# MiNeves00/SR-GAN-FD

Hardware: AMD Instinct MI355X
Metric: SR training images/sec (128->512 x4, f16) (higher is better)
Workload: dtype f16; 1 GPU; BSRGAN RRDBNet x4 generator-only (L1), 23 RRDB, batch 32/GPU, 128->512; global_batch=32, num_rrdb=23, parallelism=dp1

## Files before the change

sr_gan_fd_amd/csrc/pack.hip:

```cpp
#include "common.hpp"

namespace srganfd {

__global__ __launch_bounds__(256) void pack_kernel(const srganfd_pack_job* __restrict__ jobs, const float* __restrict__ params,
                                                   const float* __restrict__ scalars, char* __restrict__ packed) {
  const srganfd_pack_job& J = jobs[blockIdx.y];
  const int KT = J.ksize * J.ksize;
  const long long total = (long long)KT * J.k * J.n;
  const int nChunks = J.k >> 5;
  for (long long e = (long long)blockIdx.x * 256 + threadIdx.x; e < total; e += (long long)gridDim.x * 256) {
    int lane, s, k_in, within = (int)(e & 1023);
    long long blk = e >> 10;
    const int tap = (int)(blk % KT); blk /= KT;
    const int chunk = (int)(blk % nChunks);
    const int ntile = (int)(blk / nChunks);
    int n_in = -1;
    if (J.dtype != SRGANFD_F32 && J.layout == 1) {
      const int j = within & 7; lane = (within >> 3) & 63; s = within >> 9;
      k_in = 8 * (lane >> 4) + j;
      n_in = 16 * s + (lane & 15);
    } else if (J.dtype != SRGANFD_F32) {
      const int j = within & 7; lane = (within >> 3) & 63; s = within >> 9;
      k_in = 16 * s + 8 * (lane >> 5) + j;
    } else {
      lane = within & 63; s = within >> 6;
      k_in = 2 * s + (lane >> 5);
    }
    const int k = chunk * 32 + k_in, n = ntile * 32 + (n_in >= 0 ? n_in : (lane & 31));
    float v = 0.f;
    for (int g = 0; g < J.nseg; ++g) {
      const srganfd_pack_seg& S = J.seg[g];
      if (k >= S.k_lo && k < S.k_lo + S.k_len) {
        const int kk = k - S.k_lo;
        int co, ci, t = 0;
        int KTs = KT;
        int ym = 0, xm = 0;
        if (!S.transposed) { co = n + S.co_off; ci = kk + S.ci_off; t = tap; }
        else if (S.transposed == 1) { co = kk + S.co_off; ci = n + S.ci_off; t = KT - 1 - tap; }
        else if (S.transposed < 6) {
          const int py = (S.transposed - 2) >> 1, px = (S.transposed - 2) & 1, ta = tap >> 1, tb = tap & 1;
          const int ty = py ? 2 - 2 * ta : 3 - 2 * ta, tx = px ? 2 - 2 * tb : 3 - 2 * tb;
          co = kk + S.co_off; ci = n + S.ci_off; t = ty * 4 + tx; KTs = 16;
        } else if (S.transposed < 10) {
          const int py = (S.transposed - 6) >> 1, px = (S.transposed - 6) & 1, ta = tap >> 1, tb = tap & 1;
          const int ty = py ? (ta ? 0 : 2) : (ta ? -1 : 1), tx = px ? (tb ? 0 : 2) : (tb ? -1 : 1);
          co = kk + S.co_off; ci = n + S.ci_off; KTs = 9;
          t = ty * 3 + tx;
          if (ty < 0 || tx < 0) co = S.co_src;
        } else if (S.transposed < 14) {
          const int ab = S.transposed - 10;
          co = kk + S.co_off; ci = n + S.ci_off; t = ab; KTs = 4;
        } else if (S.transposed < 18) {
          const int py = (S.transposed - 14) >> 1, px = (S.transposed - 14) & 1, ta = tap >> 1, tb = tap & 1;
          co = n + S.co_off; ci = kk + S.ci_off; KTs = 9;
          ym = py ? (ta ? 4 : 3) : (ta ? 6 : 1);
          xm = px ? (tb ? 4 : 3) : (tb ? 6 : 1);
        } else {
          const int u = tap >> 2, w = tap & 3;
          co = kk + S.co_off; ci = n + S.ci_off; KTs = 9;
          ym = (0x1364 >> (4 * u)) & 7;
          xm = (0x1364 >> (4 * w)) & 7;
        }
        if (co < S.co_src && ci < S.ci_src) {
          const float* src = params + S.src_off + ((long long)co * S.ci_src + ci) * KTs;
          if (ym) {
            float sum = 0.f;
            for (int ty = 0; ty < 3; ++ty)
              for (int tx = 0; tx < 3; ++tx)
                if ((ym >> ty) & (xm >> tx) & 1) sum += src[ty * 3 + tx];
            v = sum * S.scale;
          } else {
            v = src[t] * S.scale;
          }
          if (S.scale_off >= 0) v *= scalars[S.scale_off];
        }
        break;
      }
    }
    if (J.dtype == SRGANFD_BF16) ((bf16_t*)(packed + J.dst_off))[e] = f2bf(v);
    else if (J.dtype == SRGANFD_F16) ((f16_t*)(packed + J.dst_off))[e] = (f16_t)v;
    else ((float*)(packed + J.dst_off))[e] = v;
  }
}

extern "C" size_t srganfd_packed_bytes(int32_t dtype, int32_t ksize, int32_t k, int32_t n) {
  if (k <= 0 || n <= 0 || k % 32 || n % 32) return 0;
  return (size_t)ksize * ksize * k * n * (dtype == SRGANFD_F32 ? 4 : 2);
}
extern "C" int srganfd_pack_weights(const srganfd_pack_job* jobs_dev, int32_t njobs, int64_t max_elems, const float* params,
                                    const float* scalars, void* packed, void* stream) {
  if (!jobs_dev || njobs <= 0 || max_elems <= 0 || !params || !packed) return set_err(SRGANFD_EINVAL, "pack_weights: bad args");
  long long gx = (max_elems + 255) / 256;
  if (gx > 4096) gx = 4096;
  SRGANFD_LAUNCH(pack_kernel, dim3((unsigned)gx, (unsigned)njobs), dim3(256), 0, (hipStream_t)stream, jobs_dev, params, scalars, (char*)packed);
  SRGANFD_HIP_CHECK(hipGetLastError());
  return SRGANFD_OK;
}

}
```

Before: 551.4 img/s.

## Tile weight packing through shared memory with coalesced source loads and vector stores

The weight pack kernel now processes one 32x32 (k,n) block per workgroup. It stages the source weight rows for that block into LDS with coalesced reads, then emits 16-byte vectorized stores per thread. The goal is to replace the scattered per-element global gathers of the fp32 master weights during each step's repack. It adds LDS use and two barriers per block, and changes the grid sizing. An environment variable can turn the tiling off.

```diff
diff --git a/sr_gan_fd_amd/csrc/pack.hip b/sr_gan_fd_amd/csrc/pack.hip
--- a/sr_gan_fd_amd/csrc/pack.hip
+++ b/sr_gan_fd_amd/csrc/pack.hip
@@ -1,87 +1,168 @@
 #include "common.hpp"
+#include <cstdlib>
 
 namespace srganfd {
 
-__global__ __launch_bounds__(256) void pack_kernel(const srganfd_pack_job* __restrict__ jobs, const float* __restrict__ params,
-                                                   const float* __restrict__ scalars, char* __restrict__ packed) {
-  const srganfd_pack_job& J = jobs[blockIdx.y];
-  const int KT = J.ksize * J.ksize;
-  const long long total = (long long)KT * J.k * J.n;
-  const int nChunks = J.k >> 5;
-  for (long long e = (long long)blockIdx.x * 256 + threadIdx.x; e < total; e += (long long)gridDim.x * 256) {
-    int lane, s, k_in, within = (int)(e & 1023);
-    long long blk = e >> 10;
-    const int tap = (int)(blk % KT); blk /= KT;
-    const int chunk = (int)(blk % nChunks);
-    const int ntile = (int)(blk / nChunks);
-    int n_in = -1;
-    if (J.dtype != SRGANFD_F32 && J.layout == 1) {
-      const int j = within & 7; lane = (within >> 3) & 63; s = within >> 9;
-      k_in = 8 * (lane >> 4) + j;
-      n_in = 16 * s + (lane & 15);
-    } else if (J.dtype != SRGANFD_F32) {
-      const int j = within & 7; lane = (within >> 3) & 63; s = within >> 9;
-      k_in = 16 * s + 8 * (lane >> 5) + j;
-    } else {
-      lane = within & 63; s = within >> 6;
-      k_in = 2 * s + (lane >> 5);
-    }
-    const int k = chunk * 32 + k_in, n = ntile * 32 + (n_in >= 0 ? n_in : (lane & 31));
-    float v = 0.f;
-    for (int g = 0; g < J.nseg; ++g) {
-      const srganfd_pack_seg& S = J.seg[g];
-      if (k >= S.k_lo && k < S.k_lo + S.k_len) {
-        const int kk = k - S.k_lo;
-        int co, ci, t = 0;
-        int KTs = KT;
-        int ym = 0, xm = 0;
-        if (!S.transposed) { co = n + S.co_off; ci = kk + S.ci_off; t = tap; }
-        else if (S.transposed == 1) { co = kk + S.co_off; ci = n + S.ci_off; t = KT - 1 - tap; }
-        else if (S.transposed < 6) {
-          const int py = (S.transposed - 2) >> 1, px = (S.transposed - 2) & 1, ta = tap >> 1, tb = tap & 1;
-          const int ty = py ? 2 - 2 * ta : 3 - 2 * ta, tx = px ? 2 - 2 * tb : 3 - 2 * tb;
-          co = kk + S.co_off; ci = n + S.ci_off; t = ty * 4 + tx; KTs = 16;
-        } else if (S.transposed < 10) {
-          const int py = (S.transposed - 6) >> 1, px = (S.transposed - 6) & 1, ta = tap >> 1, tb = tap & 1;
-          const int ty = py ? (ta ? 0 : 2) : (ta ? -1 : 1), tx = px ? (tb ? 0 : 2) : (tb ? -1 : 1);
-          co = kk + S.co_off; ci = n + S.ci_off; KTs = 9;
-          t = ty * 3 + tx;
-          if (ty < 0 || tx < 0) co = S.co_src;
-        } else if (S.transposed < 14) {
-          const int ab = S.transposed - 10;
-          co = kk + S.co_off; ci = n + S.ci_off; t = ab; KTs = 4;
-        } else if (S.transposed < 18) {
-          const int py = (S.transposed - 14) >> 1, px = (S.transposed - 14) & 1, ta = tap >> 1, tb = tap & 1;
-          co = n + S.co_off; ci = kk + S.ci_off; KTs = 9;
-          ym = py ? (ta ? 4 : 3) : (ta ? 6 : 1);
-          xm = px ? (tb ? 4 : 3) : (tb ? 6 : 1);
-        } else {
-          const int u = tap >> 2, w = tap & 3;
-          co = kk + S.co_off; ci = n + S.ci_off; KTs = 9;
-          ym = (0x1364 >> (4 * u)) & 7;
-          xm = (0x1364 >> (4 * w)) & 7;
-        }
-        if (co < S.co_src && ci < S.ci_src) {
-          const float* src = params + S.src_off + ((long long)co * S.ci_src + ci) * KTs;
-          if (ym) {
+static constexpr int kPackTileTaps = 9;
+static constexpr int kPackRow = 32 * kPackTileTaps + 1;
+
+__device__ __forceinline__ void pack_pos(int dtype, int layout, int within, int& k_in, int& n_in) {
+  if (dtype != SRGANFD_F32 && layout == 1) {
+    const int j = within & 7, lane = (within >> 3) & 63, s = within >> 9;
+    k_in = 8 * (lane >> 4) + j;
+    n_in = 16 * s + (lane & 15);
+  } else if (dtype != SRGANFD_F32) {
+    const int j = within & 7, lane = (within >> 3) & 63, s = within >> 9;
+    k_in = 16 * s + 8 * (lane >> 5) + j;
+    n_in = lane & 31;
+  } else {
+    const int lane = within & 63, s = within >> 6;
+    k_in = 2 * s + (lane >> 5);
+    n_in = lane & 31;
+  }
+}
+
+struct PackSrc { int co, ci, t, KTs, ym, xm; };
+__device__ __forceinline__ PackSrc pack_source(const srganfd_pack_seg& S, int KT, int tap, int kk, int n) {
+  PackSrc P;
+  P.t = 0; P.KTs = KT; P.ym = 0; P.xm = 0;
+  if (!S.transposed) { P.co = n + S.co_off; P.ci = kk + S.ci_off; P.t = tap; }
+  else if (S.transposed == 1) { P.co = kk + S.co_off; P.ci = n + S.ci_off; P.t = KT - 1 - tap; }
+  else if (S.transposed < 6) {
+    const int py = (S.transposed - 2) >> 1, px = (S.transposed - 2) & 1, ta = tap >> 1, tb = tap & 1;
+    const int ty = py ? 2 - 2 * ta : 3 - 2 * ta, tx = px ? 2 - 2 * tb : 3 - 2 * tb;
+    P.co = kk + S.co_off; P.ci = n + S.ci_off; P.t = ty * 4 + tx; P.KTs = 16;
+  } else if (S.transposed < 10) {
+    const int py = (S.transposed - 6) >> 1, px = (S.transposed - 6) & 1, ta = tap >> 1, tb = tap & 1;
+    const int ty = py ? (ta ? 0 : 2) : (ta ? -1 : 1), tx = px ? (tb ? 0 : 2) : (tb ? -1 : 1);
+    P.co = kk + S.co_off; P.ci = n + S.ci_off; P.KTs = 9;
+    P.t = ty * 3 + tx;
+    if (ty < 0 || tx < 0) P.co = S.co_src;
+  } else if (S.transposed < 14) {
+    const int ab = S.transposed - 10;
+    P.co = kk + S.co_off; P.ci = n + S.ci_off; P.t = ab; P.KTs = 4;
+  } else if (S.transposed < 18) {
+    const int py = (S.transposed - 14) >> 1, px = (S.transposed - 14) & 1, ta = tap >> 1, tb = tap & 1;
+    P.co = n + S.co_off; P.ci = kk + S.ci_off; P.KTs = 9;
+    P.ym = py ? (ta ? 4 : 3) : (ta ? 6 : 1);
+    P.xm = px ? (tb ? 4 : 3) : (tb ? 6 : 1);
+  } else {
+    const int u = tap >> 2, w = tap & 3;
+    P.co = kk + S.co_off; P.ci = n + S.ci_off; P.KTs = 9;
+    P.ym = (0x1364 >> (4 * u)) & 7;
+    P.xm = (0x1364 >> (4 * w)) & 7;
+  }
+  return P;
+}
+__device__ __forceinline__ int pack_src_taps(int transposed, int KT) {
+  return transposed < 2 ? KT : transposed < 6 ? 16 : transposed < 10 ? 9 : transposed < 14 ? 4 : 9;
+}
+__device__ __forceinline__ bool pack_co_is_n(int transposed) { return transposed == 0 || (transposed >= 14 && transposed < 18); }
+
+__device__ __forceinline__ float pack_element(const srganfd_pack_job& J, int KT, int tap, int k, int n, const float* __restrict__ params,
+                                              const float* __restrict__ scalars, const float* tile, int tile_seg, int co0, int ci0) {
+  float v = 0.f;
+  for (int g = 0; g < J.nseg; ++g) {
+    const srganfd_pack_seg& S = J.seg[g];
+    if (k >= S.k_lo && k < S.k_lo + S.k_len) {
+      const PackSrc P = pack_source(S, KT, tap, k - S.k_lo, n);
+      if (P.co < S.co_src && P.ci < S.ci_src) {
+        auto value = [&](const float* src) __attribute__((always_inline)) {
+          if (P.ym) {
             float sum = 0.f;
             for (int ty = 0; ty < 3; ++ty)
               for (int tx = 0; tx < 3; ++tx)
-                if ((ym >> ty) & (xm >> tx) & 1) sum += src[ty * 3 + tx];
-            v = sum * S.scale;
-          } else {
-            v = src[t] * S.scale;
+                if ((P.ym >> ty) & (P.xm >> tx) & 1) sum += src[ty * 3 + tx];
+            return sum * S.scale;
           }
-          if (S.scale_off >= 0) v *= scalars[S.scale_off];
-        }
-        break;
+          return src[P.t] * S.scale;
+        };
+        if (g == tile_seg) v = value(tile + (P.co - co0) * kPackRow + (P.ci - ci0) * P.KTs);
+        else v = value(params + S.src_off + ((long long)P.co * S.ci_src + P.ci) * P.KTs);
+        if (S.scale_off >= 0) v *= scalars[S.scale_off];
       }
+      break;
     }
-    if (J.dtype == SRGANFD_BF16) ((bf16_t*)(packed + J.dst_off))[e] = f2bf(v);
-    else if (J.dtype == SRGANFD_F16) ((f16_t*)(packed + J.dst_off))[e] = (f16_t)v;
-    else ((float*)(packed + J.dst_off))[e] = v;
+  }
+  return v;
+}
+
+template <typename T>
+__device__ __forceinline__ void pack_store16(const srganfd_pack_job& J, int KT, int tap, int within0, int k0, int n0, long long e0,
+                                             const float* __restrict__ params, const float* __restrict__ scalars, char* __restrict__ packed,
+                                             const float* tile, int tile_seg, int co0, int ci0) {
+  constexpr int VEC = 16 / (int)sizeof(T);
+  float v[VEC];
+#pragma unroll
+  for (int j = 0; j < VEC; ++j) {
+    int k_in, n_in;
+    pack_pos(J.dtype, J.layout, within0 + j, k_in, n_in);
+    v[j] = pack_element(J, KT, tap, k0 + k_in, n0 + n_in, params, scalars, tile, tile_seg, co0, ci0);
+  }
+  u32x4* dst = (u32x4*)(packed + J.dst_off + e0 * (long long)sizeof(T));
+  if constexpr (sizeof(T) == 2) *dst = pack8<T>(v);
+  else *dst = u32x4{__float_as_uint(v[0]), __float_as_uint(v[1]), __float_as_uint(v[2]), __float_as_uint(v[3])};
+}
+
+__global__ __launch_bounds__(256) void pack_kernel(const srganfd_pack_job* __restrict__ jobs, const float* __restrict__ params,
+                                                   const float* __restrict__ scalars, char* __restrict__ packed, int tiled) {
+  __shared__ float tile[32 * kPackRow];
+  const srganfd_pack_job& J = jobs[blockIdx.y];
+  const int KT = J.ksize * J.ksize;
+  const int nChunks = J.k >> 5;
+  const int nblocks = nChunks * (J.n >> 5);
+  const int tid = threadIdx.x;
+  for (int b = blockIdx.x; b < nblocks; b += gridDim.x) {
+    const int chunk = b % nChunks, ntile = b / nChunks;
+    const int k0 = chunk * 32, n0 = ntile * 32;
+    int sg = -1;
+    for (int g = 0; g < J.nseg; ++g)
+      if (k0 >= J.seg[g].k_lo && k0 + 32 <= J.seg[g].k_lo + J.seg[g].k_len) { sg = g; break; }
+    int co0 = 0, ci0 = 0;
+    if (!tiled || (sg >= 0 && pack_src_taps(J.seg[sg].transposed, KT) > kPackTileTaps)) sg = -1;
+    if (sg >= 0) {
+      const srganfd_pack_seg& S = J.seg[sg];
+      const int KTs = pack_src_taps(S.transposed, KT);
+      const bool co_n = pack_co_is_n(S.transposed);
+      co0 = (co_n ? n0 : k0 - S.k_lo) + S.co_off;
+      ci0 = (co_n ? k0 - S.k_lo : n0) + S.ci_off;
+      const int run = min(32, S.ci_src - ci0) * KTs;
+      const float* __restrict__ base = params + S.src_off + ((long long)co0 * S.ci_src + ci0) * KTs;
+      constexpr int kFill = 32 * 32 * kPackTileTaps / 256;
+      const int rowlen = 32 * KTs, rows = min(32, S.co_src - co0);
+      const unsigned mdiv = (65536u + KTs - 1) / KTs;
+      const long long pitch = (long long)S.ci_src * KTs;
+      float v[kFill];
+#pragma unroll
+      for (int i = 0; i < kFill; ++i) {
+        const int f = tid + i * 256;
+        const int r = (int)(((unsigned)(f >> 5) * mdiv) >> 16), c = f - r * rowlen;
+        v[i] = (r < rows && c < run) ? base[r * pitch + c] : 0.f;
+      }
+      __syncthreads();
+#pragma unroll
+      for (int i = 0; i < kFill; ++i) {
+        const int f = tid + i * 256;
+        const int r = (int)(((unsigned)(f >> 5) * mdiv) >> 16), c = f - r * rowlen;
+        if (r < 32) tile[r * kPackRow + c] = v[i];
+      }
+      __syncthreads();
+    }
+    const long long eb = (long long)b * KT * 1024;
+    if (J.dtype == SRGANFD_F32) {
+      for (int q = tid; q < KT * 256; q += 256)
+        pack_store16<float>(J, KT, q >> 8, (q & 255) * 4, k0, n0, eb + (long long)q * 4, params, scalars, packed, tile, sg, co0, ci0);
+    } else if (J.dtype == SRGANFD_BF16) {
+      for (int q = tid; q < KT * 128; q += 256)
+        pack_store16<bf16_t>(J, KT, q >> 7, (q & 127) * 8, k0, n0, eb + (long long)q * 8, params, scalars, packed, tile, sg, co0, ci0);
+    } else {
+      for (int q = tid; q < KT * 128; q += 256)
+        pack_store16<f16_t>(J, KT, q >> 7, (q & 127) * 8, k0, n0, eb + (long long)q * 8, params, scalars, packed, tile, sg, co0, ci0);
+    }
   }
 }
+
+static const bool g_pack_tiled = [] { const char* e = getenv("SRGANFD_PACK_TILED"); return !(e && e[0] == '0'); }();
 
 extern "C" size_t srganfd_packed_bytes(int32_t dtype, int32_t ksize, int32_t k, int32_t n) {
   if (k <= 0 || n <= 0 || k % 32 || n % 32) return 0;
@@ -90,9 +171,12 @@
 extern "C" int srganfd_pack_weights(const srganfd_pack_job* jobs_dev, int32_t njobs, int64_t max_elems, const float* params,
                                     const float* scalars, void* packed, void* stream) {
   if (!jobs_dev || njobs <= 0 || max_elems <= 0 || !params || !packed) return set_err(SRGANFD_EINVAL, "pack_weights: bad args");
-  long long gx = (max_elems + 255) / 256;
+  long long gx = (max_elems + 1023) / 1024;
+  const long long per_job = 8192 / njobs > 16 ? 8192 / njobs : 16;
+  if (gx > per_job) gx = per_job;
   if (gx > 4096) gx = 4096;
-  SRGANFD_LAUNCH(pack_kernel, dim3((unsigned)gx, (unsigned)njobs), dim3(256), 0, (hipStream_t)stream, jobs_dev, params, scalars, (char*)packed);
+  SRGANFD_LAUNCH(pack_kernel, dim3((unsigned)gx, (unsigned)njobs), dim3(256), 0, (hipStream_t)stream, jobs_dev, params, scalars, (char*)packed,
+                 g_pack_tiled ? 1 : 0);
   SRGANFD_HIP_CHECK(hipGetLastError());
   return SRGANFD_OK;
 }
```

Result: slower. 545.8 img/s (-1.0%).
